# waffcloud/sitewhere

Measured on AMD Instinct MI355X. Metric: device_events_per_sec, higher is better.
Workload: dtype fp64/int64 (event values as in the reference; no reduced precision)

## Files before the change

### csrc/hip/swgpu.hip

```cpp
#include <hip/hip_runtime.h>
#include <hsa/hsa.h>
#include <hsa/hsa_ext_amd.h>
#include <stdint.h>
#include "swtypes.h"
#include "swdecode.h"
#include "swengine.h"
#include "swseg.h"
#include "swblock.h"

#define BLK 256
#define WAVES (BLK / 64)
#define TILE_ITEMS 4
#define TILE (BLK * TILE_ITEMS)
#define MAX_GRID 2048
#define STAGE_BYTES (32 * 1024)
#define MAX_PROBE 4096

#ifndef SW_XCD_REMAP
#define SW_XCD_REMAP 0
#endif
__device__ __forceinline__ uint32_t sw_block_id() {
#if SW_XCD_REMAP
  const uint32_t nwg = gridDim.x, orig = blockIdx.x, x = orig % 8u, q = nwg / 8u, r = nwg % 8u;
  return (x < r ? x * (q + 1u) : r * (q + 1u) + (x - r) * q) + orig / 8u;
// ... 124 lines not shown
}

__device__ __forceinline__ bool stage_window(const uint8_t* __restrict__ raw, const uint32_t* __restrict__ off,
                                             int64_t n_msgs, uint8_t* lds, uint32_t* base_abs) {
  const int64_t m0 = (int64_t)BID * BLK;
  int64_t m1 = m0 + BLK;
  if (m1 > n_msgs) m1 = n_msgs;
  const uint32_t s = off[m0], e = off[m1];
  const uint32_t a0 = s & ~15u;
  const uint32_t span = e - a0;
  if (span > STAGE_BYTES) return false;
  const uint32_t nvec = (span + 15) >> 4;
  const uint4* src = reinterpret_cast<const uint4*>(raw + a0);
  uint4* dst = reinterpret_cast<uint4*>(lds);
  for (uint32_t v = threadIdx.x; v < nvec; v += BLK) dst[v] = src[v];
  __syncthreads();
  *base_abs = a0;
  return true;
}

#define CNT_ERR 0x80000000u
#define CNT_OVR 0x40000000u

__global__ __launch_bounds__(BLK) void k_decode_count(const uint8_t* __restrict__ raw, const uint32_t* __restrict__ off,
                                                      int64_t n_msgs, uint32_t* __restrict__ cnt,
                                                      uint32_t* __restrict__ tsum, SwEngineArgs a) {
  __shared__ __attribute__((aligned(16))) uint8_t lds[STAGE_BYTES];
  if (BID == 0 && threadIdx.x == 0) {
    *a.n_new_names = 0;
    *a.overflow = 0;
    ((ull*)a.stats)[SW_STAT_MSGS] += (ull)a.n_msgs;
  }
  uint32_t base = 0;
  const bool staged = stage_window(raw, off, n_msgs, lds, &base);
  __shared__ uint32_t red[WAVES + 1];
  const int64_t m = (int64_t)BID * BLK + threadIdx.x;
  uint32_t c = 0;
  if (m < n_msgs) {
    uint32_t verdict = SW_DEC_UNKNOWN;
    c = staged ? sw_decode_payload(lds, off[m] - base, off[m + 1] - base, base, 0, 0, nullptr, 0, &verdict)
               : sw_decode_payload(raw, off[m], off[m + 1], 0, 0, 0, nullptr, 0, &verdict);
    cnt[m] = c | (verdict == SW_DEC_ERROR ? CNT_ERR : 0u) | (verdict == SW_DEC_OVERSIZE ? CNT_OVR : 0u);
  }
  uint32_t tot;
  block_excl_scan(c, &tot, red);
  if (threadIdx.x == 0) tsum[BID] = tot;
}

__device__ __forceinline__ void note_name(const SwEventRec& r, ull* __restrict__ key, int64_t mask,
                                          SwNameRef* __restrict__ list, uint32_t* __restrict__ n_list, int64_t cap) {
  if (r.name_hash == 0 || r.etype >= 16) return;
  const ull h = r.name_hash;
  int64_t slot = (int64_t)(h & (ull)mask);
  for (int64_t p = 0; p <= mask && p < MAX_PROBE; ++p) {
    ull old = key[slot];
    if (old == h) return;
    if (old == 0) {
      old = atomicCAS(&key[slot], 0ull, h);
      if (old == 0) {
        const uint32_t k = atomicAdd(n_list, 1u);
        if (k < cap) {
          SwNameRef ref;
          ref.hash = h; ref.off = r.aux_off; ref.len = r.aux_len; ref.src_rank = r.src_rank; ref.pad = r.etype;
          list[k] = ref;
        } else {
          atomicExch(&key[slot], 0ull);
        }
        return;
      }
      if (old == h) return;
    }
    slot = (slot + 1) & mask;
  }
}

__global__ __launch_bounds__(BLK) void k_decode_emit(SwEngineArgs a) {
  __shared__ __attribute__((aligned(16))) uint8_t lds[STAGE_BYTES];
  uint32_t base = 0;
  const bool staged = stage_window(a.raw, a.msg_off, a.n_msgs, lds, &base);
  __shared__ uint32_t red[WAVES + 1];
  const int64_t m = (int64_t)BID * BLK + threadIdx.x;
  uint32_t tot;
  const uint32_t cv = m < a.n_msgs ? a.msg_cnt[m] : 0u;
  const uint32_t pre = block_excl_scan(cv & ~(CNT_ERR | CNT_OVR), &tot, red);
  const uint32_t blk_off = block_sum_prefix(a.msg_evoff, BID, red);
  if (BID == 0) {
    const uint32_t all = block_sum_prefix(a.msg_evoff, gridDim.x, red);
    if (threadIdx.x == 0) *a.n_recs = all;
  }
  if (m >= a.n_msgs) return;
  uint32_t verdict = (cv & CNT_ERR) ? SW_DEC_ERROR : (cv & CNT_OVR) ? SW_DEC_OVERSIZE : SW_DEC_VALID;
  const int64_t o = (int64_t)blk_off + pre;
  if (o >= a.rec_cap) return;
  const uint32_t room = (uint32_t)((a.rec_cap - o) < 0xffffffffll ? (a.rec_cap - o) : 0xffffffffll);
  SwEventRec* out = a.recs + o;
  uint32_t n;
  SwStrRef* sp = a.spans ? a.spans + o : nullptr;
  if (staged)
    n = sw_decode_payload(lds, a.msg_off[m] - base, a.msg_off[m + 1] - base, base, a.now_ms, (uint8_t)a.rank, out, room,
                          &verdict, sp);
// ... 673 lines not shown
      }
    }
    ok += __popcll(__ballot(v && st == SW_ST_OK));
    all += __popcll(__ballot(v));
    if (st != SW_ST_OK) atomicAdd(&rs[st & 7], 1u);
  }
  if (lane_id() == 0) { atomicAdd(&c[0], ok); atomicAdd(&c[1], all - ok); }
  __syncthreads();
  if (threadIdx.x == 0) { tcnt[BID] = c[0]; tcnt[ntiles + BID] = c[1]; }
  if (threadIdx.x < 8 && rs[threadIdx.x]) {
    const int slot = threadIdx.x == SW_ST_UNREGISTERED ? SW_STAT_UNREGISTERED
                   : threadIdx.x == SW_ST_UNASSIGNED ? SW_STAT_UNASSIGNED
                   : threadIdx.x == SW_ST_DUPLICATE ? SW_STAT_DUPLICATE
                   : threadIdx.x == SW_ST_DECODE_ERROR ? SW_STAT_DECODE_ERROR
                   : threadIdx.x == SW_ST_CONTROL ? SW_STAT_CONTROL
                   : threadIdx.x == SW_ST_RECHECK ? SW_STAT_DEDUP_RECHECKS : -1;
    if (slot >= 0) atomicAdd(&stats[slot], (ull)rs[threadIdx.x]);
  }
}

__global__ void k_cmp_write(const uint8_t* __restrict__ status, const uint32_t* __restrict__ n_ptr,
                            const uint32_t* __restrict__ tcnt, int64_t ntiles,
                            uint32_t* __restrict__ ok_idx, uint32_t* __restrict__ rej_idx,
                            uint32_t* __restrict__ n_ok, uint32_t* __restrict__ n_rej) {
  __shared__ uint32_t lds[WAVES + 1];
  const uint32_t n = *n_ptr;
  const int64_t base = (int64_t)BID * TILE;
  uint32_t run_ok = block_sum_prefix(tcnt, BID, lds);
  uint32_t run_rj = block_sum_prefix(tcnt + ntiles, BID, lds);
  if (BID == gridDim.x - 1 && threadIdx.x == 0) {
    *n_ok = run_ok + tcnt[BID];
    *n_rej = run_rj + tcnt[ntiles + BID];
  }
  for (int k = 0; k < TILE_ITEMS; ++k) {
    const int64_t i = base + (int64_t)k * BLK + threadIdx.x;
    const bool valid = i < n;
    const bool ok = valid && status[i] == SW_ST_OK;
    const bool rj = valid && !ok;
    uint32_t tot_ok, tot_rj;
    uint32_t p_ok = block_excl_scan(ok ? 1u : 0u, &tot_ok, lds);
    uint32_t p_rj = block_excl_scan(rj ? 1u : 0u, &tot_rj, lds);
    if (ok) ok_idx[run_ok + p_ok] = (uint32_t)i;
    if (rj) rej_idx[run_rj + p_rj] = (uint32_t)i;
    run_ok += tot_ok;
    run_rj += tot_rj;
  }
}

template <typename K>
__device__ __forceinline__ int64_t nm_probe(const K* __restrict__ key, int64_t mask, ull h) {
  int64_t slot = (int64_t)(h & (ull)mask);
  for (int64_t p = 0; p <= mask && p < MAX_PROBE; ++p) {
    const ull k = key[slot];
    if (k == h) return slot;
    if (k == 0) return -1;
    slot = (slot + 1) & mask;
  }
  return -1;
}

__global__ void k_intern_insert_list(const SwEventRec* __restrict__ recs, const uint32_t* __restrict__ n_ptr,
                                     ull* __restrict__ key, int32_t* __restrict__ ids, int32_t* __restrict__ counter,
                                     int64_t mask, uint32_t cap) {
  const uint32_t n = *n_ptr < cap ? *n_ptr : cap;
  for (int64_t j = (int64_t)BID * BLK + threadIdx.x; j < n; j += (int64_t)gridDim.x * BLK)
    if (recs[j].name_hash) intern_insert(key, ids, counter, mask, recs[j].name_hash);
}

__device__ __forceinline__ int64_t ms_slot(SwMsSlot* __restrict__ ms, int64_t mask, ull k) {
  int64_t slot = (int64_t)(sw_mix64(k) & (ull)mask);
  for (int64_t p = 0; p <= mask && p < MAX_PROBE; ++p) {
    ull* kp = (ull*)&ms[slot].key;
    ull old = *kp;
    if (old == k) return slot;
    if (old == 0) {
      old = atomicCAS(kp, 0ull, k);
      if (old == 0 || old == k) return slot;
    }
    slot = (slot + 1) & mask;
  }
  return -1;
}

__global__ void k_persist(SwEngineArgs a, const SwEventRec* __restrict__ R, const uint32_t* __restrict__ idx,
                          const int32_t* __restrict__ devs, const int32_t* __restrict__ asgs,
                          const uint32_t* __restrict__ n_ptr, uint32_t cap, const SwStrRef* __restrict__ spans,
                          const uint32_t* __restrict__ after) {
  const uint32_t n = *n_ptr < cap ? *n_ptr : cap;
  const int64_t cur = *a.store_cursor + (after ? (int64_t)*after : 0);
  if (idx && BID == 0 && threadIdx.x == 0) {
    if (a.dd_meta[1] + a.rec_cap > (a.dd_mask + 1) / 2) a.dd_meta[2] = 1;
  }
  uint32_t ff_ids = 0;
  const int64_t c0 = *a.step_cursor0;
  const int64_t now = a.sp->now_ms;
  SwSegAux* const aux = reinterpret_cast<SwSegAux*>(a.sp->aux);
  const int64_t raw_bytes = a.sp->raw_bytes;
  for (int64_t j = (int64_t)BID * BLK + threadIdx.x; j < n; j += (int64_t)gridDim.x * BLK) {
    const uint32_t i = idx ? idx[j] : (uint32_t)j;
    const SwEventRec r = R[i];
    const int32_t dev = devs[i], asg = asgs[i];
    const int64_t seq = cur + j;
    const int64_t row = seq % a.store_cap;
    a.s_etype[row] = r.etype;
    a.s_level[row] = r.level;
    a.s_date[row] = r.event_date;
    a.s_recv[row] = now;
    a.s_dev[row] = dev;
    a.s_asg[row] = asg;
    const int4 ctx = *reinterpret_cast<const int4*>(&a.asg_ctx[asg]);
    a.s_cust[row] = ctx.y;
    a.s_area[row] = ctx.z;
    a.s_asset[row] = ctx.w;
    a.s_name[row] = r.name_hash;
    a.s_v0[row] = r.v0;
    a.s_v1[row] = r.v1;
    a.s_v2[row] = r.v2;
    a.s_alt[row] = r.alt_hash;
    a.s_aux[row] = ((ull)r.src_rank << 48) | ((ull)r.aux_len << 32) | (ull)r.aux_off;
    a.s_batch[row] = (int32_t)a.sp->batch_seq;
    SwOutRec o;
    o.event_date = r.event_date;
    o.v0 = r.v0;
    o.v1 = r.v1;
// ... 326 lines not shown
}

__global__ void k_presence(SwEngineArgs a) {
  const SwStepParams P = *a.sp;
  if (P.presence_missing_ms <= 0) return;
  const ull limit = (ull)(P.now_ms - P.presence_missing_ms);
  for (int64_t s = (int64_t)BID * BLK + threadIdx.x; s < a.n_asg; s += (int64_t)gridDim.x * BLK) {
    SwAsgState* st = &a.st[s];
    const ull last = st->last;
    const bool miss = last != 0 && last < limit && st->missing == 0 && a.asg_active[s];
    if (!miss) continue;
    st->missing = (ull)P.now_ms;
    const uint32_t g = atomicAdd(a.n_gen, 1u);
    if (g < a.gen_cap) {
      SwEventRec r;
      r.fp_lo = 0; r.fp_hi = 0; r.event_date = P.now_ms; r.name_hash = a.presence_name_hash;
      r.v0 = 0; r.v1 = 0; r.v2 = 0; r.alt_hash = 0;
      r.aux_off = 0; r.aux2_off = 0; r.aux_len = 0; r.aux2_len = 0;
      r.etype = SW_EV_STATE_CHANGE; r.flags = 0; r.src_rank = (uint8_t)a.rank; r.level = 0;
      a.gen[g] = r;
      a.gen_dev[g] = a.asg_ctx[s].device;
      a.gen_asg[g] = (int32_t)s;
    }
  }
}

__global__ void k_decode_begin(SwEngineArgs a) {
  if (threadIdx.x == 0 && BID == 0) {
    *a.n_new_names = 0;
    *a.overflow = 0;
    ((ull*)a.stats)[SW_STAT_MSGS] += (ull)a.n_msgs;
  }
}

__global__ void k_gen_clamp(SwEngineArgs a, uint32_t* gen_rules) {
  if (threadIdx.x == 0 && BID == 0) {
    if (*a.n_gen > a.gen_cap) *a.n_gen = (uint32_t)a.gen_cap;
    if (gen_rules) *gen_rules = *a.n_gen;
  }
}

__global__ void k_step_end(SwEngineArgs a, const uint32_t* n_rule_alerts) {
  if (threadIdx.x == 0 && BID == 0) {
    if (*a.n_gen > a.gen_cap) *a.n_gen = (uint32_t)a.gen_cap;
    *a.store_cursor += (int64_t)*a.n_ok + *a.n_gen;
    *a.n_out = (uint32_t)(*a.store_cursor - *a.step_cursor0);
    *a.seq_base += *a.n_work;
    ull* st = (ull*)a.stats;
    st[SW_STAT_EVENTS] += *a.n_work;
    st[SW_STAT_PERSISTED] += *a.n_out;
    st[SW_STAT_RULE_ALERTS] += *n_rule_alerts;
    st[SW_STAT_PRESENCE] += *a.n_gen - *n_rule_alerts;
    int64_t* meta = a.dd_meta;
    if (meta[2] == 1) {
// ... 784 lines not shown

int sw_step_snapshot(const uint32_t* scalars, const uint32_t* seg_meta, const uint32_t* rej_cnt,
                     const uint32_t* n_carry, int32_t produced, SwStepSnapshot* host, hipStream_t s) {
  k_step_snapshot<<<1, 64, 0, s>>>(scalars, seg_meta, rej_cnt, n_carry, produced, host);
  return (int)hipGetLastError();
}

int sw_frame_varint(const uint8_t* lens, int64_t nbytes, int64_t n_msgs, uint32_t* msg_off, uint32_t raw_bytes,
                    uint32_t* tmp, int64_t tmp_len, hipStream_t s) {
  int64_t nt = (nbytes + TILE - 1) / TILE;
  if (nt < 1) nt = 1;
  if (2 * nt > tmp_len) return -2;
  if (nbytes <= 0 || n_msgs <= 0) return (int)hipMemsetAsync(msg_off, 0, sizeof(uint32_t) * (n_msgs + 1), s);
  uint32_t* tcnt = tmp;
  uint32_t* tlen = tmp + nt;
  k_vlen_tiles<<<(unsigned)nt, BLK, 0, s>>>(lens, nbytes, tcnt, tlen);
  k_vlen_apply<<<(unsigned)nt, BLK, 0, s>>>(lens, nbytes, tcnt, tlen, msg_off, n_msgs, raw_bytes);
  return (int)hipGetLastError();
}

int sw_phase_decode(const SwEngineArgs* ap, hipStream_t s) {
  const SwEngineArgs a = *ap;
  if (a.n_msgs <= 0) {
    k_decode_begin<<<1, 64, 0, s>>>(a);
    (void)hipMemsetAsync(a.n_recs, 0, sizeof(uint32_t), s);
    return (int)hipGetLastError();
  }
  const unsigned nb = (unsigned)((a.n_msgs + BLK - 1) / BLK);
  k_decode_count<<<nb, BLK, 0, s>>>(a.raw, a.msg_off, a.n_msgs, a.msg_cnt, a.msg_evoff, a);
  k_decode_emit<<<nb, BLK, 0, s>>>(a);
  if (a.world > 1) k_decode_end<<<1, 64, 0, s>>>(a);
  return (int)hipGetLastError();
}

int sw_phase_partition(const SwEngineArgs* ap, hipStream_t s) {
  const SwEngineArgs a = *ap;
  const int64_t ntiles = (a.carry_cap + a.rec_cap + TILE - 1) / TILE;
  if (a.world > 64 || ntiles * a.world > a.part_tmp_len || !a.carry || !a.n_carry || !a.spill || !a.n_spill ||
      a.carry == a.spill || !a.part_owner || !a.part_bytes || !a.part_meta || ntiles >= 0x7fffffff)
    return -3;
  if (a.send_str && (!a.part_len || !a.carry_spans || !a.carry_str || !a.spill_spans || !a.spill_str ||
                     a.carry_str == a.spill_str || a.carry_str_cap <= 0 || a.carry_str_cap > 0xffffffffll ||
                     a.str_cap > 0x7fffffffll))
    return -4;
  k_part_count<<<(unsigned)ntiles, BLK, 0, s>>>(a.carry, a.n_carry, a.recs, a.n_recs, (int)a.world, (int)a.rank,
                                                a.part_tmp, ntiles, a);
  int rc = launch_scan(a.part_tmp, ntiles * a.world, a.part_tmp + ntiles * a.world, nullptr, a.scan_tmp,
                       a.scan_tmp_len, s);
  if (rc) return rc;
  const uint32_t* toff = a.part_tmp + ntiles * a.world;
  k_part_cut<<<(unsigned)a.world, BLK, 0, s>>>(toff, a.part_tmp, ntiles, a.n_carry, a.n_recs, a);
  k_part_write<<<(unsigned)ntiles, BLK, 0, s>>>(a.carry, a.n_carry, a.recs, a.n_recs, (int)a.world, (int)a.rank, toff,
                                                a.part_tmp, ntiles, a.send, a.shuf_cap, a.spill, a.carry_cap, a);
  k_part_counts<<<1, 64, 0, s>>>(toff, a.part_tmp, ntiles, (int)a.world, a);
  return (int)hipGetLastError();
}

int sw_phase_unpack(const SwEngineArgs* ap, hipStream_t s) {
  const SwEngineArgs a = *ap;
  if (a.work_str && (a.str_cap & 15)) return -5;
  k_unpack<<<grid_for(a.rec_cap), BLK, 0, s>>>(a.recv, a.recv_cnt, (int)a.world, a.shuf_cap, a.work, a.n_work,
                                               a.rec_cap, a);
  return (int)hipGetLastError();
}

__global__ void k_cl_prep(const uint32_t* __restrict__ ok_idx, const uint32_t* __restrict__ n_ok,
                          const int32_t* __restrict__ ev_asg, uint32_t* __restrict__ keys, uint32_t* __restrict__ vals) {
  const uint32_t n = *n_ok;
  for (int64_t j = (int64_t)BID * BLK + threadIdx.x; j < n; j += (int64_t)gridDim.x * BLK) {
    const uint32_t i = ok_idx[j];
    keys[j] = (uint32_t)ev_asg[i];
    vals[j] = i;
  }
}

__global__ __launch_bounds__(BLK) void k_ff_add_rows(SwEngineArgs a, const SwEventRec* __restrict__ R,
                                                     const uint32_t* __restrict__ idx,
                                                     const uint32_t* __restrict__ n_ptr, uint32_t cap) {
  if (!a.dd_ff) return;
  const uint32_t n = *n_ptr < cap ? *n_ptr : cap;
  uint32_t* __restrict__ t = a.dd_ff;
  const int gens = (int)a.dd_ff_gens, g = (int)a.dd_ff_meta[0];
  const int64_t bmask = a.dd_ff_bmask;
  const uint32_t lane = threadIdx.x & 63u, sub = lane & 3u, grp = lane >> 2;
  const ull gmask = 0xfull << (4u * grp);
  const int64_t g0 = ((int64_t)BID * BLK + threadIdx.x) >> 2;
  const int64_t gstride = ((int64_t)gridDim.x * BLK) >> 2;
  uint32_t dropped = 0;
  for (int64_t base = g0 - grp; base < (int64_t)n; base += gstride) {
    const int64_t j = base + grp;
    ull h = 0ull;
    if (j < (int64_t)n) h = R[idx ? idx[j] : (uint32_t)j].alt_hash;
    const ull m = sw_ff_mix(h);
    const uint32_t fp = sw_ff_fp(m);
    int64_t b = (int64_t)sw_ff_bucket(m, bmask);
    bool pending = h != 0ull;
    for (int p = 0; p < 2 * SW_FF_MAX_PROBE && __any(pending); ++p) {
      uint32_t* sl = t + (b * gens + g) * SW_FF_SLOTS;
      uint4 v = make_uint4(1u, 1u, 1u, 1u);
      if (pending) v = reinterpret_cast<const uint4*>(sl)[sub];
      const bool hit = pending && (v.x == fp || v.y == fp || v.z == fp || v.w == fp);
      if (__ballot(hit) & gmask) pending = false;
      const bool zero = pending && (!v.x || !v.y || !v.z || !v.w);
      const ull zb = __ballot(zero) & gmask;
      bool ok = false;
      if (pending && zb && lane == (uint32_t)(__ffsll((long long)zb) - 1)) {
        const int k = !v.x ? 0 : !v.y ? 1 : !v.z ? 2 : 3;
        const uint32_t old = atomicCAS(&sl[4u * sub + (uint32_t)k], 0u, fp);
        ok = old == 0u || old == fp;
      }
      if (__ballot(ok) & gmask) pending = false;
      else if (pending && !zb) b = (b + 1) & bmask;
    }
    if (pending && sub == 0u) ++dropped;
  }
  if (dropped) atomicAdd((ull*)&a.dd_ff_meta[5], (ull)dropped);
}

int sw_phase_process(const SwEngineArgs* ap, uint32_t* scratch4, hipStream_t s) {
  const SwEngineArgs a = *ap;
  const int g = grid_for(a.rec_cap);
  const int64_t ntiles = (a.rec_cap + TILE - 1) / TILE;
  if (2 * ntiles > a.scan_tmp_len) return -4;
  if (a.dd_ff && (a.dd_ff_gens < 2 || a.dd_ff_gens > SW_FF_MAX_GENS || !a.dd_ff_meta || a.dd_ff_bmask < 0))
    return -6;
  if (a.n_mtests < 0 || (a.n_mtests > 0 && (!a.mtests || a.n_tests + a.n_mtests > ZONE_LDS_TESTS))) return -7;
  k_lookup<<<g, BLK, 0, s>>>(a);
  if (a.dd_ff) k_ff_probe<<<g, BLK, 0, s>>>(a);
  k_dedup_claim<<<g, BLK, 0, s>>>(a);
  k_cmp_count<<<(unsigned)ntiles, BLK, 0, s>>>(a.status, a.n_work, a.cmp_tmp, ntiles, (ull*)a.stats, a.work,
                                               (const ull*)a.dd_key, a.dd_mask, a.seq_base, a.dd_meta,
                                               a.dd_ff, a.dd_ff_bmask, (int)a.dd_ff_gens, a.work_str ? -1 : (int)a.rank);
  k_cmp_write<<<(unsigned)ntiles, BLK, 0, s>>>(a.status, a.n_work, a.cmp_tmp, ntiles, a.ok_idx, a.rej_idx, a.n_ok,
                                               a.n_rej);
  int rc = 0;
  if (a.cl_bits > 0) {
    k_cl_prep<<<g, BLK, 0, s>>>(a.ok_idx, a.n_ok, a.ev_asg, a.cl_keys, a.cl_vals);
    rc = sw_radix_sort_u32(a.cl_keys, a.cl_vals, a.n_ok, a.rec_cap, (int)a.cl_bits, a.cl_hist, a.ok_idx, s);
    if (rc < 0) return rc;
  }
  const SwStrRef* wsp = a.world > 1 ? a.work_spans : a.spans;
  k_persist<<<g, BLK, 0, s>>>(a, a.work, a.ok_idx, a.ev_dev, a.ev_asg, a.n_ok, (uint32_t)a.rec_cap, wsp, nullptr);
  if (a.dd_ff) k_ff_add_rows<<<g, BLK, 0, s>>>(a, a.work, a.ok_idx, a.n_ok, (uint32_t)a.rec_cap);
  k_state_p2<<<g, BLK, 0, s>>>(a, a.n_ok, (uint32_t)a.rec_cap, nullptr);
  uint32_t* n_rule = scratch4;
  if (a.n_tests + a.n_mtests > 0) {
    const int64_t otiles = (a.rec_cap + TILE - 1) / TILE;
    ull* zmask = (ull*)a.zmask;
    uint32_t* ztile = a.ztile;
    if (a.n_tests > 0) {
      const size_t vtx_bytes = zone_vtx_in_lds(a) ? (size_t)a.n_zone_vtx * 2 * sizeof(double) : 0;
      k_zone_mask<<<(unsigned)otiles, BLK, vtx_bytes, s>>>(a, zmask, ztile);
    }
    if (a.n_mtests > 0) k_mx_mask<<<(unsigned)otiles, BLK, 0, s>>>(a, zmask, ztile, a.n_tests > 0 ? 0 : 1);
    k_zone_emit<<<(unsigned)otiles, BLK, 0, s>>>(a, zmask, ztile, n_rule);
  } else {
    k_gen_clamp<<<1, 64, 0, s>>>(a, n_rule);
  }
  k_presence<<<grid_for(a.n_asg), BLK, 0, s>>>(a);
  const int gg = grid_for(a.gen_cap);
  const uint32_t gcap = (uint32_t)a.gen_cap;
  k_intern_insert_list<<<gg, BLK, 0, s>>>(a.gen, a.n_gen, (ull*)a.nm_key, a.nm_id, a.nm_counter, a.nm_mask, gcap);
  k_persist<<<gg, BLK, 0, s>>>(a, a.gen, nullptr, a.gen_dev, a.gen_asg, a.n_gen, gcap, nullptr, a.n_ok);
  if (a.dd_ff) k_ff_add_rows<<<gg, BLK, 0, s>>>(a, a.gen, nullptr, a.n_gen, gcap);
  k_state_p2<<<gg, BLK, 0, s>>>(a, a.n_gen, gcap, a.n_ok);
  k_step_end<<<1, 64, 0, s>>>(a, n_rule);
  return (int)hipGetLastError();
}

__global__ void k_set_step_params(SwStepParams* sp, int64_t now_ms, int64_t batch_seq, int64_t presence_ms,
                                  SwOutRec* out, void* aux, int64_t raw_bytes) {
  if (threadIdx.x == 0 && BID == 0) {
    sp->now_ms = now_ms; sp->batch_seq = batch_seq; sp->presence_missing_ms = presence_ms; sp->out = out;
    sp->aux = aux; sp->raw_bytes = raw_bytes;
  }
}

__global__ void k_ff_add(uint32_t* t, int64_t bmask, int gens, int g, int64_t* meta, const ull* __restrict__ h,
                         int64_t n) {
  uint32_t dropped = 0;
  for (int64_t i = (int64_t)BID * BLK + threadIdx.x; i < n; i += (int64_t)gridDim.x * BLK)
    if (h[i] && !ff_add(t, bmask, gens, g, h[i])) ++dropped;
  if (dropped) atomicAdd((ull*)&meta[5], (ull)dropped);
}

__global__ void k_ff_clear(uint32_t* t, int64_t bmask, int gens, int g) { ff_clear_gen(t, bmask, gens, g); }

// ... 342 lines not shown
```

### csrc/include/swdecode.h

```cpp
#pragma once
#include "swtypes.h"

SW_HD void sw_fill_control(SwEventRec* r, uint8_t etype, uint32_t abs_start, uint32_t abs_end,
                           uint64_t lo, uint64_t hi, int64_t now_ms, uint8_t src_rank) {
  r->fp_lo = lo; r->fp_hi = hi; r->event_date = now_ms; r->name_hash = 0;
  r->v0 = 0; r->v1 = 0; r->v2 = 0; r->alt_hash = 0;
  r->aux_off = abs_start; r->aux2_off = abs_end; r->aux_len = 0; r->aux2_len = 0;
  r->etype = etype; r->flags = 0; r->src_rank = src_rank; r->level = 0;
}

SW_HD void sw_clear_span(SwStrRef* s) {
  s->alt_off = 0; s->meta_off = 0; s->alt_len = 0; s->meta_len = 0; s->k = 0; s->has = 0; s->pad = 0;
}

SW_HD bool sw_read_tag(const uint8_t* buf, uint32_t* pos, uint32_t end, uint32_t* f, uint32_t* wt) {
  uint64_t key;
  if (!sw_read_varint(buf, pos, end, &key) || key > 0xffffffffull || (key >> 3) == 0) return false;
  *f = (uint32_t)(key >> 3);
  *wt = (uint32_t)(key & 7);
  return true;
}

SW_HD bool sw_check_pair(const uint8_t* buf, uint32_t* pos, uint32_t end, uint32_t wt2, uint32_t* len1 = nullptr) {
  uint64_t len;
// ... 7 lines not shown
    const uint32_t vs = p;
    if (!sw_skip_field(buf, &p, e, wt)) return false;
    if (f == 1 && wt == 2) {
      h1 = true;
      if (len1) {
        uint32_t q = vs;
        uint64_t l;
        sw_read_varint(buf, &q, e, &l);
        if ((uint32_t)l > *len1) *len1 = (uint32_t)l;
      }
    }
    h2 |= f == 2 && wt == wt2;
  }
  *pos = e;
  return h1 && h2;
}

#define SW_DEC_UNKNOWN 0u
#define SW_DEC_VALID 1u
#define SW_DEC_ERROR 2u
#define SW_DEC_OVERSIZE 3u
SW_HD uint32_t sw_decode_payload(const uint8_t* buf, uint32_t start, uint32_t end, uint32_t abs_base,
                                 int64_t now_ms, uint8_t src_rank, SwEventRec* out, uint32_t max_out,
                                 uint32_t* verdict = nullptr, SwStrRef* spans = nullptr) {
  const uint32_t known = verdict ? *verdict : SW_DEC_UNKNOWN;
  if (out && known == SW_DEC_ERROR) {
    if (max_out) {
      sw_fill_control(out, SW_EV_DECODE_ERROR, abs_base + start, abs_base + end, 0, 0, now_ms, src_rank);
      if (spans) sw_clear_span(spans);
    }
    return 1;
  }
  const bool trusted = out && known == SW_DEC_VALID;
  uint32_t pos = start;
  uint64_t hlen = 0, blen = 0, v = 0;
  uint64_t cmd = 0;
  bool ok = sw_read_varint(buf, &pos, end, &hlen) && hlen <= (uint64_t)(end - pos);
  if (ok) {
    uint32_t hend = pos + (uint32_t)hlen;
    while (ok && pos < hend) {
      uint32_t f, wt;
      ok = sw_read_tag(buf, &pos, hend, &f, &wt);
      if (!ok) break;
      if (f == 1 && wt == 0) {
        ok = sw_read_varint(buf, &pos, hend, &v);
        if (v >= 1 && v <= 8) cmd = v;
      } else {
        ok = sw_skip_field(buf, &pos, hend, wt);
      }
    }
    ok = ok && sw_read_varint(buf, &pos, end, &blen) && blen <= (uint64_t)(end - pos);
  }
  if (!ok || cmd < 1 || cmd > 8) {
    if (out && max_out) {
      sw_fill_control(out, SW_EV_DECODE_ERROR, abs_base + start, abs_base + end, 0, 0, now_ms, src_rank);
      if (spans) sw_clear_span(spans);
    }
    if (!out && verdict) *verdict = SW_DEC_ERROR;
    return 1;
  }
  const uint32_t bstart = pos, bend = pos + (uint32_t)blen;
  const bool event = cmd == SW_CMD_SEND_DEVICE_MEASUREMENTS || cmd == SW_CMD_SEND_DEVICE_LOCATION ||
                     cmd == SW_CMD_SEND_DEVICE_ALERT;
  const uint32_t meta_f = cmd == SW_CMD_SEND_DEVICE_MEASUREMENTS ? 4u : cmd == SW_CMD_SEND_DEVICE_LOCATION ? 6u : 5u;

  uint64_t lo = 0, hi = 0, date = 0;
  bool has_dev = false, has_date = false, has_us = false, us = false, has_elev = false, has_alt = false;
  bool req_a = false, req_b = false;
  uint32_t n_mx = 0, name_max = 0;
  double lat = 0, lon = 0, elev = 0;
  uint32_t t_off = start, t_len = 0, m_off = start, m_len = 0;
  uint32_t a_off = start, a_len = 0;
  uint32_t md_lo = 0, md_hi = 0;
  bool has_md = false;
  pos = bstart;
  while (ok && pos < bend) {
    uint32_t f, wt;
    const uint32_t fstart = pos;
    ok = sw_read_tag(buf, &pos, bend, &f, &wt);
    if (!ok) break;
    if (f == 1 && wt == 2) {
// ... 34 lines not shown
          if (f == 2) { lat = d; req_a = true; } else if (f == 3) { lon = d; req_b = true; }
          else if (f == 4) { elev = d; has_elev = true; }
          else { date = bits; has_date = true; }
        } else if (f == 7 && wt == 0) { ok = sw_read_varint(buf, &pos, bend, &v); has_us = true; us = v != 0; }
        else ok = sw_skip_field(buf, &pos, bend, wt);
        break;
      case SW_CMD_SEND_DEVICE_ALERT:
        if ((f == 2 || f == 3) && wt == 2) {
          ok = sw_read_varint(buf, &pos, bend, &v) && v <= (uint64_t)(bend - pos);
          if (!ok) break;
          if (f == 2) { t_off = pos; t_len = (uint32_t)v; req_a = true; } else { m_off = pos; m_len = (uint32_t)v; req_b = true; }
          pos += (uint32_t)v;
        } else if (f == 4 && wt == 1) { if (pos + 8 > bend) { ok = false; break; } date = sw_load_le64(buf + pos); pos += 8; has_date = true; }
        else if (f == 6 && wt == 0) { ok = sw_read_varint(buf, &pos, bend, &v); has_us = true; us = v != 0; }
        else ok = sw_skip_field(buf, &pos, bend, wt);
        break;
      default:
        ok = sw_skip_field(buf, &pos, bend, wt);
        break;
    }
  }
  if ((cmd == SW_CMD_SEND_DEVICE_LOCATION || cmd == SW_CMD_SEND_DEVICE_ALERT) && !(req_a && req_b)) ok = false;
  if (!ok || !has_dev) {
    if (!out && verdict) *verdict = SW_DEC_ERROR;
    if (out && max_out) {
      sw_fill_control(out, SW_EV_DECODE_ERROR, abs_base + start, abs_base + end, 0, 0, now_ms, src_rank);
      if (spans) sw_clear_span(spans);
    }
    return 1;
  }
  const bool oversize = event && (known == SW_DEC_OVERSIZE ||
                                  (!trusted && (a_len > 0xffffu || md_hi - md_lo > 0xffffu || t_len > 0xffffu ||
                                                m_len > 0xffffu || name_max > 0xffffu)));
  if (oversize) {
    if (!out && verdict) *verdict = SW_DEC_OVERSIZE;
    if (!out) return 1;
    if (!max_out) return 0;
    sw_fill_control(out, SW_EV_OVERSIZE, abs_base + start, abs_base + end, lo, hi, now_ms, src_rank);
    if (spans) sw_clear_span(spans);
    return 1;
  }
  uint8_t flags = (has_us ? SW_F_HAS_UPDATE_STATE : 0) | (us ? SW_F_UPDATE_STATE : 0) |
                  (has_date ? SW_F_HAS_DATE : 0) | (has_elev ? SW_F_HAS_ELEVATION : 0);
  int64_t edate = has_date ? (int64_t)date : now_ms;
  SwStrRef sp;
  sp.alt_off = abs_base + a_off; sp.alt_len = (uint16_t)a_len;
  sp.meta_off = has_md ? abs_base + md_lo : abs_base + start; sp.meta_len = has_md ? (uint16_t)(md_hi - md_lo) : 0;
  sp.k = 0; sp.has = (has_alt ? SW_SR_ALT : 0) | (has_md ? SW_SR_META : 0); sp.pad = 0;

  if (!out && verdict) *verdict = SW_DEC_VALID;
  if (!out) return cmd == SW_CMD_SEND_DEVICE_MEASUREMENTS ? n_mx : 1;
  const uint64_t alt = has_alt && (cmd != SW_CMD_SEND_DEVICE_MEASUREMENTS || n_mx == 1) ? sw_hash64(buf + a_off, a_len) : 0;
  if (cmd == SW_CMD_SEND_DEVICE_MEASUREMENTS) {
    if (n_mx > max_out) {
      if (max_out) {
        sw_fill_control(out, SW_EV_DECODE_ERROR, abs_base + start, abs_base + end, lo, hi, now_ms, src_rank);
        if (spans) sw_clear_span(spans);
      }
      return max_out ? 1 : 0;
    }
    const bool multi = n_mx > 1;
    uint32_t k = 0;
    pos = bstart;
    while (pos < bend && k < n_mx) {
      uint64_t key;
      if (!sw_read_varint(buf, &pos, bend, &key)) break;
      uint32_t f = (uint32_t)(key >> 3), wt = (uint32_t)(key & 7);
      if (!(f == 2 && wt == 2)) { if (!sw_skip_field(buf, &pos, bend, wt)) break; continue; }
      sw_read_varint(buf, &pos, bend, &v);
      uint32_t mend = pos + (uint32_t)v;
      uint32_t n_off = start, n_len = 0;
      double val = 0;
      while (pos < mend) {
        uint64_t k2;
// ... 62 lines not shown
```

### csrc/include/swengine.h

```cpp
#pragma once
#include <stddef.h>
#include <stdint.h>
#include "swtypes.h"

typedef struct SwNameRef {
  uint64_t hash;
  uint32_t off;
  uint16_t len;
  uint8_t src_rank;
  uint8_t pad;
} SwNameRef;

typedef struct __attribute__((aligned(16))) SwRegSlot {
  uint64_t lo;
  uint64_t hi;
  int32_t dev;
  int32_t asg;
  uint64_t pad;
} SwRegSlot;

typedef struct __attribute__((aligned(16))) SwAsgCtx {
  int32_t device;
  int32_t customer;
  int32_t area;
// ... 138 lines not shown
  const SwStrRef* recv_spans;
  uint8_t* work_str;
  SwStrRef* work_spans;
  int64_t str_cap;
  uint32_t* str_drops;
  uint8_t* part_owner;
  uint32_t* cl_keys;
  uint32_t* cl_vals;
  uint32_t* cl_hist;
  int64_t cl_bits;
  uint32_t* part_len;
  uint64_t* part_bytes;
  uint64_t* part_meta;
  const SwStrRef* carry_spans;
  const uint8_t* carry_str;
  SwStrRef* spill_spans;
  uint8_t* spill_str;
  uint32_t* n_spill_str;
  int64_t carry_str_cap;
  const SwMxTest* mtests;
  int64_t n_mtests;
} SwEngineArgs;

enum {
  SW_SC_N_RECS = 0,
  SW_SC_N_NEW_NAMES,
  SW_SC_OVERFLOW,
  SW_SC_N_WORK,
  SW_SC_N_OK,
  SW_SC_N_REJ,
  SW_SC_N_GEN,
  SW_SC_N_OUT,
  SW_SC_N_RULE,
  SW_SC_WORDS = 16,
};

typedef struct SwStepSnapshot {
  uint32_t scalars[SW_SC_WORDS];
  uint64_t block_bytes, block_errors, block_first_seq;
  uint32_t n_carry[2];
  uint32_t rej_refs, rej_bytes;
  uint32_t pad[6];
} SwStepSnapshot;
static_assert(sizeof(SwStepSnapshot) == 128, "SwStepSnapshot is 32 u32 words");
static_assert(offsetof(SwStepSnapshot, block_bytes) == 64 && offsetof(SwStepSnapshot, n_carry) == 88 &&
              offsetof(SwStepSnapshot, rej_refs) == 96, "SwStepSnapshot layout");
// ... 139 lines not shown
```

### sitewhere_amd/models/columnar.py

```python
from __future__ import annotations

import numpy as np

EV_MEASUREMENT = 0
EV_LOCATION = 1
EV_ALERT = 2
EV_COMMAND_INVOCATION = 3
EV_COMMAND_RESPONSE = 4
EV_STATE_CHANGE = 5
EV_REGISTRATION = 16
EV_ACK = 17
EV_STREAM_CREATE = 18
EV_STREAM_DATA = 19
EV_STREAM_DATA_REQUEST = 20
EV_DECODE_ERROR = 255

ST_OK = 0
ST_UNREGISTERED = 1
ST_UNASSIGNED = 2
ST_DUPLICATE = 3
ST_DECODE_ERROR = 4
ST_CONTROL = 5
ST_RECHECK = 6

# ... 58 lines not shown

OUT_REC = np.dtype([
    ("event_date", "<i8"), ("v0", "<f8"), ("v1", "<f8"), ("assignment", "<i4"), ("name_id", "<u2"),
    ("etype", "u1"), ("level", "u1"),
])
OUT_REC_SIZE = 32
assert OUT_REC.itemsize == OUT_REC_SIZE
NO_NAME = 0xFFFF

NAME_REF = np.dtype([("hash", "<u8"), ("off", "<u4"), ("len", "<u2"), ("src_rank", "u1"), ("etype", "u1")])
assert NAME_REF.itemsize == 16

REG_SLOT = np.dtype([("lo", "<u8"), ("hi", "<u8"), ("dev", "<i4"), ("asg", "<i4"), ("pad", "<u8")])
assert REG_SLOT.itemsize == 32
ASG_STATE = np.dtype([("last", "<u8"), ("missing", "<u8"), ("loc_date", "<u8"), ("loc_eid1", "<u8")])
MS_SLOT = np.dtype([("key", "<u8"), ("date", "<u8"), ("eid1", "<u8"), ("pad", "<u8")])

ZONE_TEST = np.dtype([("zone", "<i4"), ("condition", "<i4"), ("alert_name_id", "<i4"), ("level", "<i4")])
MX_TEST = np.dtype([("name_hash", "<u8"), ("lo", "<f8"), ("hi", "<f8")])

SC_NAMES = ("n_recs", "n_new_names", "overflow", "n_work", "n_ok", "n_rej", "n_gen", "n_out", "n_rule")
SC_N_RECS, SC_N_NEW_NAMES, SC_OVERFLOW, SC_N_WORK, SC_N_OK, SC_N_REJ, SC_N_GEN, SC_N_OUT, SC_N_RULE = range(9)
SC_WORDS = 16

STEP_SNAPSHOT = np.dtype([
    ("scalars", "<u4", (SC_WORDS,)), ("block_bytes", "<u8"), ("block_errors", "<u8"), ("block_first_seq", "<u8"),
    ("n_carry", "<u4", (2,)), ("rej_refs", "<u4"), ("rej_bytes", "<u4"), ("pad", "<u4", (6,)),
])
assert STEP_SNAPSHOT.itemsize == 128

SERIES_CELL = np.dtype([
    ("count", "<i8"), ("sum", "<f8"), ("min", "<f8"), ("max", "<f8"), ("first", "<f8"), ("last", "<f8"),
    ("first_date", "<i8"), ("last_date", "<i8"), ("first_id", "<i8"), ("last_id", "<i8"),
])
assert SERIES_CELL.itemsize == 80
SERIES_MAX_NAMES = 64
SERIES_MAX_CELLS = 65536
RING_QUERY = ("etype", "asg", "date", "n_rows", "seq0", "head", "bits", "n_asg", "start", "end")
SERIES_QUERY = RING_QUERY + ("name", "v0", "names", "n_names", "bucket_ms", "n_buckets", "rounds", "grid")
NEAR_QUERY = RING_QUERY + ("v0", "v1", "lat", "lon", "radius_m", "lat_lo", "lat_hi", "lon_lo", "lon_hi", "latest",
                           "best_date", "best_seq")
NEAR_QUERY_F64 = ("lat", "lon", "radius_m", "lat_lo", "lat_hi", "lon_lo", "lon_hi")
ZONE_QUERY = RING_QUERY + ("v0", "v1", "vtx", "n_vtx", "lat_lo", "lat_hi", "lon_lo", "lon_hi", "outside", "latest",
                           "best_date", "best_seq")
ZONE_QUERY_F64 = ("lat_lo", "lat_hi", "lon_lo", "lon_hi")
GRID_CELL = np.dtype([("count", "<i8"), ("last_date", "<i8")])
# ... 30 lines not shown
```

### sitewhere_amd/pipeline/gpu_engine.py

```python
from __future__ import annotations

import ctypes
import functools
import os
import time

import numpy as np
import torch

from .._native import gpu_gil as gpu_lib
from ..models.columnar import (EVENT_REC, RANK_CELL, RANK_QUERY, GRID_CELL, GRID_QUERY_F64, GRID_WORDS, N_STATS, NEAR_QUERY, NEAR_QUERY_F64,
                               OUT_REC, NAME_REF, OUT_REC_SIZE, RING_QUERY, SC_N_GEN, SC_N_NEW_NAMES, SC_N_OK, SC_N_OUT,
                               SC_N_RECS, SC_N_REJ, SC_N_RULE, SC_N_WORK, SC_NAMES, SC_OVERFLOW, SEG_ST_BYTES, SEG_ST_FIRST, SEG_ST_WORDS, SERIES_CELL, SERIES_QUERY,
                               ST_RECHECK, STEP_SNAPSHOT, STR_REF, WIRE_REC, ZONE_QUERY, ZONE_QUERY_F64)
from ..ops.engine_abi import SwEngineArgs
from .config import EngineConfig
from .bus_io import host_view
from .engine_base import EngineBase, StepResult
from .pinned_pool import PinnedPool

_ALIGN = 64
_I64 = np.iinfo(np.int64)


def _ptr(t: torch.Tensor) -> int:
    return t.data_ptr()


def _chk(rc: int, name: str):
    if rc:
        raise RuntimeError(f"{name} failed ({rc})")


class HostBuffer:
# ... 541 lines not shown
        return self.t["recv"][q * n:(q + 1) * n]

    def loopback_strings(self, peers: list):
        c = self.cfg
        if not c.str_cap:
            return
        sr = c.shuf_cap * STR_REF.itemsize
        q = self.rank
        for r, e in enumerate(peers):
            p = e._last_send_par
            self.t["recv_str_cnt"][r] = e.send_str_cnts[p][q]
            self.t["recv_spans"][r * sr:(r + 1) * sr].copy_(e.send_spans[p][q * sr:(q + 1) * sr])
            self.t["recv_str"][r * c.str_cap:(r + 1) * c.str_cap].copy_(
                e.send_strs[p][q * c.str_cap:(q + 1) * c.str_cap])

    def string_drops(self) -> dict:
        v = self.t["str_drops"].cpu().numpy()
        return {"oversize": int(v[0])}

    def scalars(self) -> dict:
        v = self.t["scalars"][:len(SC_NAMES)].cpu().numpy()
        return {name: int(x) for name, x in zip(SC_NAMES, v)}

    def step(self, raw: np.ndarray, offs: np.ndarray, now_ms: int, presence: bool | None = None) -> StepResult:
        n_msgs = len(offs) - 1
        with self._lock:
            self._no_framed_pending()
            raw_dev, off_dev = self._stage(raw, offs)
            do_presence = self.presence_due(now_ms) if presence is None else presence
            sel = self.step_async(raw_dev, off_dev, n_msgs, now_ms, presence=do_presence, out_to_device=True)
            self._sync_streams()
            return self._with_block(self.collect(sel, raw, from_device=True), sel, now_ms)

    def decode_only(self, raw: np.ndarray, offs: np.ndarray, now_ms: int, spans: bool = False):
        n_msgs = len(offs) - 1
        with self._lock:
            self._no_framed_pending()
            raw_dev, off_dev = self._stage(raw, offs)
            self._set_batch(raw_dev, off_dev, n_msgs, now_ms)
            _chk(self.lib.sw_phase_decode(ctypes.byref(self.args), self._stream()), "sw_phase_decode")
            self._sync_streams()
            n = min(int(self.t["scalars"][SC_N_RECS].item()), self.cfg.rec_cap)
            recs = self.t["recs"][:n * EVENT_REC.itemsize].cpu().numpy().view(EVENT_REC).copy()
            if not spans:
                return recs
            return recs, self.t["spans"][:n * STR_REF.itemsize].cpu().numpy().view(STR_REF).copy()
# ... 1159 lines not shown
```

Before: 523.4 million.

## Speculate single-event decode in one pass and fold cluster prep into compaction

Decoding now speculates that every message yields exactly one event. The first kernel decodes straight into the output records and only runs the two-pass emit kernel when some block saw a message with a different count. A small mode state machine on the device tracks recent fallbacks across batches so later batches use the classic path after one misses. Separately, the cluster key/value preparation kernel is merged into the compaction write, persist reads the sorted assignment keys directly, and the generated-event bloom-add launch is dropped in favour of reading alt hashes back from the store ring. These changes cut a full decode pass and several launches per step, at the cost of extra state and wasted speculative work when a batch contains multi-event messages.

```diff
diff --git a/csrc/hip/swgpu.hip b/csrc/hip/swgpu.hip
--- a/csrc/hip/swgpu.hip
+++ b/csrc/hip/swgpu.hip
@@ -170,30 +170,7 @@
 #define CNT_ERR 0x80000000u
 #define CNT_OVR 0x40000000u
 
-__global__ __launch_bounds__(BLK) void k_decode_count(const uint8_t* __restrict__ raw, const uint32_t* __restrict__ off,
-                                                      int64_t n_msgs, uint32_t* __restrict__ cnt,
-                                                      uint32_t* __restrict__ tsum, SwEngineArgs a) {
-  __shared__ __attribute__((aligned(16))) uint8_t lds[STAGE_BYTES];
-  if (BID == 0 && threadIdx.x == 0) {
-    *a.n_new_names = 0;
-    *a.overflow = 0;
-    ((ull*)a.stats)[SW_STAT_MSGS] += (ull)a.n_msgs;
-  }
-  uint32_t base = 0;
-  const bool staged = stage_window(raw, off, n_msgs, lds, &base);
-  __shared__ uint32_t red[WAVES + 1];
-  const int64_t m = (int64_t)BID * BLK + threadIdx.x;
-  uint32_t c = 0;
-  if (m < n_msgs) {
-    uint32_t verdict = SW_DEC_UNKNOWN;
-    c = staged ? sw_decode_payload(lds, off[m] - base, off[m + 1] - base, base, 0, 0, nullptr, 0, &verdict)
-               : sw_decode_payload(raw, off[m], off[m + 1], 0, 0, 0, nullptr, 0, &verdict);
-    cnt[m] = c | (verdict == SW_DEC_ERROR ? CNT_ERR : 0u) | (verdict == SW_DEC_OVERSIZE ? CNT_OVR : 0u);
-  }
-  uint32_t tot;
-  block_excl_scan(c, &tot, red);
-  if (threadIdx.x == 0) tsum[BID] = tot;
-}
+__device__ __forceinline__ uint32_t* dec_mode(const SwEngineArgs& a) { return a.n_recs + SW_SC_DECODE_MODE; }
 
 __device__ __forceinline__ void note_name(const SwEventRec& r, ull* __restrict__ key, int64_t mask,
                                           SwNameRef* __restrict__ list, uint32_t* __restrict__ n_list, int64_t cap) {
@@ -222,8 +199,62 @@
   }
 }
 
+__global__ void k_decode_begin(SwEngineArgs a, int classic) {
+  if (threadIdx.x == 0 && BID == 0) {
+    *a.n_new_names = 0;
+    *a.overflow = 0;
+    ((ull*)a.stats)[SW_STAT_MSGS] += (ull)a.n_msgs;
+    uint32_t* dm = dec_mode(a);
+    const uint32_t k = dm[SW_DM_BATCH] + 1u;
+    dm[SW_DM_BATCH] = k;
+    const bool cl = classic || dm[SW_DM_FORCE] || dm[SW_DM_W0 + (k + 2u) % 3u];
+    dm[SW_DM_W0 + (k + 1u) % 3u] = 0;
+    dm[SW_DM_MODE] = cl ? 1u : 0u;
+    if (!cl) ++dm[SW_DM_SPECULATED];
+  }
+}
+
+__global__ __launch_bounds__(BLK) void k_decode_first(SwEngineArgs a) {
+  __shared__ __attribute__((aligned(16))) uint8_t lds[STAGE_BYTES];
+  uint32_t base = 0;
+  const bool staged = stage_window(a.raw, a.msg_off, a.n_msgs, lds, &base);
+  __shared__ uint32_t red[WAVES + 1];
+  const uint32_t* dm = dec_mode(a);
+  const bool classic = dm[SW_DM_MODE] != 0u;
+  const int64_t m = (int64_t)BID * BLK + threadIdx.x;
+  uint32_t c = 0;
+  bool other = false;
+  if (m < a.n_msgs) {
+    uint32_t verdict = SW_DEC_UNKNOWN;
+    const uint32_t s = a.msg_off[m], e = a.msg_off[m + 1];
+    if (classic) {
+      c = staged ? sw_decode_payload(lds, s - base, e - base, base, 0, 0, nullptr, 0, &verdict)
+                 : sw_decode_payload(a.raw, s, e, 0, 0, 0, nullptr, 0, &verdict);
+    } else {
+      SwEventRec* out = a.recs + m;
+      SwStrRef* sp = a.spans ? a.spans + m : nullptr;
+      if (staged) sw_decode_payload(lds, s - base, e - base, base, a.now_ms, (uint8_t)a.rank, out, 1, &verdict, sp, &c);
+      else sw_decode_payload(a.raw, s, e, 0, a.now_ms, (uint8_t)a.rank, out, 1, &verdict, sp, &c);
+      if (c == 1u) note_name(*out, (ull*)a.seen_key, a.seen_mask, a.new_names, a.n_new_names, a.names_cap);
+    }
+    other = c != 1u;
+    a.msg_cnt[m] = c | (verdict == SW_DEC_ERROR ? CNT_ERR : 0u) | (verdict == SW_DEC_OVERSIZE ? CNT_OVR : 0u);
+  }
+  uint32_t tot;
+  block_excl_scan(c, &tot, red);
+  if (threadIdx.x == 0) a.msg_evoff[BID] = tot;
+  if (!classic && BID == 0 && threadIdx.x == 0) *a.n_recs = (uint32_t)a.n_msgs;
+  if (__syncthreads_or(other) && threadIdx.x == 0) dec_mode(a)[SW_DM_W0 + dm[SW_DM_BATCH] % 3u] = 1u;
+}
+
 __global__ __launch_bounds__(BLK) void k_decode_emit(SwEngineArgs a) {
   __shared__ __attribute__((aligned(16))) uint8_t lds[STAGE_BYTES];
+  {
+    uint32_t* dm = dec_mode(a);
+    const bool classic = dm[SW_DM_MODE] != 0u;
+    if (!classic && !dm[SW_DM_W0 + dm[SW_DM_BATCH] % 3u]) return;
+    if (!classic && BID == 0 && threadIdx.x == 0) ++dm[SW_DM_FALLBACKS];
+  }
   uint32_t base = 0;
   const bool staged = stage_window(a.raw, a.msg_off, a.n_msgs, lds, &base);
   __shared__ uint32_t red[WAVES + 1];
@@ -943,7 +974,9 @@
 __global__ void k_cmp_write(const uint8_t* __restrict__ status, const uint32_t* __restrict__ n_ptr,
                             const uint32_t* __restrict__ tcnt, int64_t ntiles,
                             uint32_t* __restrict__ ok_idx, uint32_t* __restrict__ rej_idx,
-                            uint32_t* __restrict__ n_ok, uint32_t* __restrict__ n_rej) {
+                            uint32_t* __restrict__ n_ok, uint32_t* __restrict__ n_rej,
+                            const int32_t* __restrict__ ev_asg, uint32_t* __restrict__ cl_keys,
+                            uint32_t* __restrict__ cl_vals) {
   __shared__ uint32_t lds[WAVES + 1];
   const uint32_t n = *n_ptr;
   const int64_t base = (int64_t)BID * TILE;
@@ -961,7 +994,14 @@
     uint32_t tot_ok, tot_rj;
     uint32_t p_ok = block_excl_scan(ok ? 1u : 0u, &tot_ok, lds);
     uint32_t p_rj = block_excl_scan(rj ? 1u : 0u, &tot_rj, lds);
-    if (ok) ok_idx[run_ok + p_ok] = (uint32_t)i;
+    if (ok) {
+      if (cl_keys) {
+        cl_keys[run_ok + p_ok] = (uint32_t)ev_asg[i];
+        cl_vals[run_ok + p_ok] = (uint32_t)i;
+      } else {
+        ok_idx[run_ok + p_ok] = (uint32_t)i;
+      }
+    }
     if (rj) rej_idx[run_rj + p_rj] = (uint32_t)i;
     run_ok += tot_ok;
     run_rj += tot_rj;
@@ -1006,7 +1046,7 @@
 __global__ void k_persist(SwEngineArgs a, const SwEventRec* __restrict__ R, const uint32_t* __restrict__ idx,
                           const int32_t* __restrict__ devs, const int32_t* __restrict__ asgs,
                           const uint32_t* __restrict__ n_ptr, uint32_t cap, const SwStrRef* __restrict__ spans,
-                          const uint32_t* __restrict__ after) {
+                          const uint32_t* __restrict__ after, const uint32_t* __restrict__ sorted_asg) {
   const uint32_t n = *n_ptr < cap ? *n_ptr : cap;
   const int64_t cur = *a.store_cursor + (after ? (int64_t)*after : 0);
   if (idx && BID == 0 && threadIdx.x == 0) {
@@ -1020,7 +1060,7 @@
   for (int64_t j = (int64_t)BID * BLK + threadIdx.x; j < n; j += (int64_t)gridDim.x * BLK) {
     const uint32_t i = idx ? idx[j] : (uint32_t)j;
     const SwEventRec r = R[i];
-    const int32_t dev = devs[i], asg = asgs[i];
+    const int32_t dev = devs[i], asg = sorted_asg ? (int32_t)sorted_asg[j] : asgs[i];
     const int64_t seq = cur + j;
     const int64_t row = seq % a.store_cap;
     a.s_etype[row] = r.etype;
@@ -1393,14 +1433,6 @@
       a.gen_dev[g] = a.asg_ctx[s].device;
       a.gen_asg[g] = (int32_t)s;
     }
-  }
-}
-
-__global__ void k_decode_begin(SwEngineArgs a) {
-  if (threadIdx.x == 0 && BID == 0) {
-    *a.n_new_names = 0;
-    *a.overflow = 0;
-    ((ull*)a.stats)[SW_STAT_MSGS] += (ull)a.n_msgs;
   }
 }
 
@@ -2231,12 +2263,13 @@
 int sw_phase_decode(const SwEngineArgs* ap, hipStream_t s) {
   const SwEngineArgs a = *ap;
   if (a.n_msgs <= 0) {
-    k_decode_begin<<<1, 64, 0, s>>>(a);
+    k_decode_begin<<<1, 64, 0, s>>>(a, 1);
     (void)hipMemsetAsync(a.n_recs, 0, sizeof(uint32_t), s);
     return (int)hipGetLastError();
   }
   const unsigned nb = (unsigned)((a.n_msgs + BLK - 1) / BLK);
-  k_decode_count<<<nb, BLK, 0, s>>>(a.raw, a.msg_off, a.n_msgs, a.msg_cnt, a.msg_evoff, a);
+  k_decode_begin<<<1, 64, 0, s>>>(a, a.rec_cap < a.n_msgs ? 1 : 0);
+  k_decode_first<<<nb, BLK, 0, s>>>(a);
   k_decode_emit<<<nb, BLK, 0, s>>>(a);
   if (a.world > 1) k_decode_end<<<1, 64, 0, s>>>(a);
   return (int)hipGetLastError();
@@ -2273,21 +2306,12 @@
   return (int)hipGetLastError();
 }
 
-__global__ void k_cl_prep(const uint32_t* __restrict__ ok_idx, const uint32_t* __restrict__ n_ok,
-                          const int32_t* __restrict__ ev_asg, uint32_t* __restrict__ keys, uint32_t* __restrict__ vals) {
-  const uint32_t n = *n_ok;
-  for (int64_t j = (int64_t)BID * BLK + threadIdx.x; j < n; j += (int64_t)gridDim.x * BLK) {
-    const uint32_t i = ok_idx[j];
-    keys[j] = (uint32_t)ev_asg[i];
-    vals[j] = i;
-  }
-}
-
 __global__ __launch_bounds__(BLK) void k_ff_add_rows(SwEngineArgs a, const SwEventRec* __restrict__ R,
                                                      const uint32_t* __restrict__ idx,
                                                      const uint32_t* __restrict__ n_ptr, uint32_t cap) {
   if (!a.dd_ff) return;
   const uint32_t n = *n_ptr < cap ? *n_ptr : cap;
+  const int64_t cur = *a.store_cursor;
   uint32_t* __restrict__ t = a.dd_ff;
   const int gens = (int)a.dd_ff_gens, g = (int)a.dd_ff_meta[0];
   const int64_t bmask = a.dd_ff_bmask;
@@ -2299,7 +2323,7 @@
   for (int64_t base = g0 - grp; base < (int64_t)n; base += gstride) {
     const int64_t j = base + grp;
     ull h = 0ull;
-    if (j < (int64_t)n) h = R[idx ? idx[j] : (uint32_t)j].alt_hash;
+    if (j < (int64_t)n) h = R ? R[idx[j]].alt_hash : a.s_alt[(cur + j) % a.store_cap];
     const ull m = sw_ff_mix(h);
     const uint32_t fp = sw_ff_fp(m);
     int64_t b = (int64_t)sw_ff_bucket(m, bmask);
@@ -2340,17 +2364,22 @@
   k_cmp_count<<<(unsigned)ntiles, BLK, 0, s>>>(a.status, a.n_work, a.cmp_tmp, ntiles, (ull*)a.stats, a.work,
                                                (const ull*)a.dd_key, a.dd_mask, a.seq_base, a.dd_meta,
                                                a.dd_ff, a.dd_ff_bmask, (int)a.dd_ff_gens, a.work_str ? -1 : (int)a.rank);
+  const bool cluster = a.cl_bits > 0;
   k_cmp_write<<<(unsigned)ntiles, BLK, 0, s>>>(a.status, a.n_work, a.cmp_tmp, ntiles, a.ok_idx, a.rej_idx, a.n_ok,
-                                               a.n_rej);
-  int rc = 0;
-  if (a.cl_bits > 0) {
-    k_cl_prep<<<g, BLK, 0, s>>>(a.ok_idx, a.n_ok, a.ev_asg, a.cl_keys, a.cl_vals);
-    rc = sw_radix_sort_u32(a.cl_keys, a.cl_vals, a.n_ok, a.rec_cap, (int)a.cl_bits, a.cl_hist, a.ok_idx, s);
+                                               a.n_rej, a.ev_asg, cluster ? a.cl_keys : nullptr, a.cl_vals);
+  const uint32_t* sorted_asg = nullptr;
+  if (cluster) {
+    const int rc = sw_radix_sort_u32(a.cl_keys, a.cl_vals, a.n_ok, a.rec_cap, (int)a.cl_bits, a.cl_hist, a.ok_idx, s);
     if (rc < 0) return rc;
+    sorted_asg = a.cl_keys + (int64_t)rc * a.rec_cap;
   }
   const SwStrRef* wsp = a.world > 1 ? a.work_spans : a.spans;
-  k_persist<<<g, BLK, 0, s>>>(a, a.work, a.ok_idx, a.ev_dev, a.ev_asg, a.n_ok, (uint32_t)a.rec_cap, wsp, nullptr);
-  if (a.dd_ff) k_ff_add_rows<<<g, BLK, 0, s>>>(a, a.work, a.ok_idx, a.n_ok, (uint32_t)a.rec_cap);
+  k_persist<<<g, BLK, 0, s>>>(a, a.work, a.ok_idx, a.ev_dev, a.ev_asg, a.n_ok, (uint32_t)a.rec_cap, wsp, nullptr,
+                              sorted_asg);
+  if (a.dd_ff) {
+    const bool ring = a.store_cap >= a.rec_cap;
+    k_ff_add_rows<<<g, BLK, 0, s>>>(a, ring ? nullptr : a.work, a.ok_idx, a.n_ok, (uint32_t)a.rec_cap);
+  }
   k_state_p2<<<g, BLK, 0, s>>>(a, a.n_ok, (uint32_t)a.rec_cap, nullptr);
   uint32_t* n_rule = scratch4;
   if (a.n_tests + a.n_mtests > 0) {
@@ -2370,8 +2399,7 @@
   const int gg = grid_for(a.gen_cap);
   const uint32_t gcap = (uint32_t)a.gen_cap;
   k_intern_insert_list<<<gg, BLK, 0, s>>>(a.gen, a.n_gen, (ull*)a.nm_key, a.nm_id, a.nm_counter, a.nm_mask, gcap);
-  k_persist<<<gg, BLK, 0, s>>>(a, a.gen, nullptr, a.gen_dev, a.gen_asg, a.n_gen, gcap, nullptr, a.n_ok);
-  if (a.dd_ff) k_ff_add_rows<<<gg, BLK, 0, s>>>(a, a.gen, nullptr, a.n_gen, gcap);
+  k_persist<<<gg, BLK, 0, s>>>(a, a.gen, nullptr, a.gen_dev, a.gen_asg, a.n_gen, gcap, nullptr, a.n_ok, nullptr);
   k_state_p2<<<gg, BLK, 0, s>>>(a, a.n_gen, gcap, a.n_ok);
   k_step_end<<<1, 64, 0, s>>>(a, n_rule);
   return (int)hipGetLastError();
diff --git a/csrc/include/swdecode.h b/csrc/include/swdecode.h
--- a/csrc/include/swdecode.h
+++ b/csrc/include/swdecode.h
@@ -53,8 +53,11 @@
 #define SW_DEC_OVERSIZE 3u
 SW_HD uint32_t sw_decode_payload(const uint8_t* buf, uint32_t start, uint32_t end, uint32_t abs_base,
                                  int64_t now_ms, uint8_t src_rank, SwEventRec* out, uint32_t max_out,
-                                 uint32_t* verdict = nullptr, SwStrRef* spans = nullptr) {
+                                 uint32_t* verdict = nullptr, SwStrRef* spans = nullptr,
+                                 uint32_t* full_cnt = nullptr) {
   const uint32_t known = verdict ? *verdict : SW_DEC_UNKNOWN;
+  const bool report = verdict && (!out || (full_cnt && known == SW_DEC_UNKNOWN));
+  if (full_cnt) *full_cnt = 1;
   if (out && known == SW_DEC_ERROR) {
     if (max_out) {
       sw_fill_control(out, SW_EV_DECODE_ERROR, abs_base + start, abs_base + end, 0, 0, now_ms, src_rank);
@@ -87,7 +90,7 @@
       sw_fill_control(out, SW_EV_DECODE_ERROR, abs_base + start, abs_base + end, 0, 0, now_ms, src_rank);
       if (spans) sw_clear_span(spans);
     }
-    if (!out && verdict) *verdict = SW_DEC_ERROR;
+    if (report) *verdict = SW_DEC_ERROR;
     return 1;
   }
   const uint32_t bstart = pos, bend = pos + (uint32_t)blen;
@@ -168,7 +171,7 @@
   }
   if ((cmd == SW_CMD_SEND_DEVICE_LOCATION || cmd == SW_CMD_SEND_DEVICE_ALERT) && !(req_a && req_b)) ok = false;
   if (!ok || !has_dev) {
-    if (!out && verdict) *verdict = SW_DEC_ERROR;
+    if (report) *verdict = SW_DEC_ERROR;
     if (out && max_out) {
       sw_fill_control(out, SW_EV_DECODE_ERROR, abs_base + start, abs_base + end, 0, 0, now_ms, src_rank);
       if (spans) sw_clear_span(spans);
@@ -179,7 +182,7 @@
                                   (!trusted && (a_len > 0xffffu || md_hi - md_lo > 0xffffu || t_len > 0xffffu ||
                                                 m_len > 0xffffu || name_max > 0xffffu)));
   if (oversize) {
-    if (!out && verdict) *verdict = SW_DEC_OVERSIZE;
+    if (report) *verdict = SW_DEC_OVERSIZE;
     if (!out) return 1;
     if (!max_out) return 0;
     sw_fill_control(out, SW_EV_OVERSIZE, abs_base + start, abs_base + end, lo, hi, now_ms, src_rank);
@@ -194,8 +197,9 @@
   sp.meta_off = has_md ? abs_base + md_lo : abs_base + start; sp.meta_len = has_md ? (uint16_t)(md_hi - md_lo) : 0;
   sp.k = 0; sp.has = (has_alt ? SW_SR_ALT : 0) | (has_md ? SW_SR_META : 0); sp.pad = 0;
 
-  if (!out && verdict) *verdict = SW_DEC_VALID;
+  if (report) *verdict = SW_DEC_VALID;
   if (!out) return cmd == SW_CMD_SEND_DEVICE_MEASUREMENTS ? n_mx : 1;
+  if (full_cnt && cmd == SW_CMD_SEND_DEVICE_MEASUREMENTS) *full_cnt = n_mx;
   const uint64_t alt = has_alt && (cmd != SW_CMD_SEND_DEVICE_MEASUREMENTS || n_mx == 1) ? sw_hash64(buf + a_off, a_len) : 0;
   if (cmd == SW_CMD_SEND_DEVICE_MEASUREMENTS) {
     if (n_mx > max_out) {
diff --git a/csrc/include/swengine.h b/csrc/include/swengine.h
--- a/csrc/include/swengine.h
+++ b/csrc/include/swengine.h
@@ -184,6 +184,17 @@
   int64_t n_mtests;
 } SwEngineArgs;
 
+#define SW_SC_DECODE_MODE 32
+enum {
+  SW_DM_BATCH = 0,
+  SW_DM_W0 = 1,
+  SW_DM_MODE = 4,
+  SW_DM_FORCE = 5,
+  SW_DM_SPECULATED = 6,
+  SW_DM_FALLBACKS = 7,
+  SW_DM_WORDS = 8,
+};
+
 enum {
   SW_SC_N_RECS = 0,
   SW_SC_N_NEW_NAMES,
diff --git a/sitewhere_amd/models/columnar.py b/sitewhere_amd/models/columnar.py
--- a/sitewhere_amd/models/columnar.py
+++ b/sitewhere_amd/models/columnar.py
@@ -104,6 +104,8 @@
 SC_NAMES = ("n_recs", "n_new_names", "overflow", "n_work", "n_ok", "n_rej", "n_gen", "n_out", "n_rule")
 SC_N_RECS, SC_N_NEW_NAMES, SC_OVERFLOW, SC_N_WORK, SC_N_OK, SC_N_REJ, SC_N_GEN, SC_N_OUT, SC_N_RULE = range(9)
 SC_WORDS = 16
+DECODE_MODE = 32
+DM_FORCE, DM_SPECULATED, DM_FALLBACKS, DM_WORDS = 5, 6, 7, 8
 
 STEP_SNAPSHOT = np.dtype([
     ("scalars", "<u4", (SC_WORDS,)), ("block_bytes", "<u8"), ("block_errors", "<u8"), ("block_first_seq", "<u8"),
diff --git a/sitewhere_amd/pipeline/gpu_engine.py b/sitewhere_amd/pipeline/gpu_engine.py
--- a/sitewhere_amd/pipeline/gpu_engine.py
+++ b/sitewhere_amd/pipeline/gpu_engine.py
@@ -9,7 +9,7 @@
 import torch
 
 from .._native import gpu_gil as gpu_lib
-from ..models.columnar import (EVENT_REC, RANK_CELL, RANK_QUERY, GRID_CELL, GRID_QUERY_F64, GRID_WORDS, N_STATS, NEAR_QUERY, NEAR_QUERY_F64,
+from ..models.columnar import (DECODE_MODE, DM_FALLBACKS, DM_FORCE, DM_SPECULATED, DM_WORDS, EVENT_REC, RANK_CELL, RANK_QUERY, GRID_CELL, GRID_QUERY_F64, GRID_WORDS, N_STATS, NEAR_QUERY, NEAR_QUERY_F64,
                                OUT_REC, NAME_REF, OUT_REC_SIZE, RING_QUERY, SC_N_GEN, SC_N_NEW_NAMES, SC_N_OK, SC_N_OUT,
                                SC_N_RECS, SC_N_REJ, SC_N_RULE, SC_N_WORK, SC_NAMES, SC_OVERFLOW, SEG_ST_BYTES, SEG_ST_FIRST, SEG_ST_WORDS, SERIES_CELL, SERIES_QUERY,
                                ST_RECHECK, STEP_SNAPSHOT, STR_REF, WIRE_REC, ZONE_QUERY, ZONE_QUERY_F64)
@@ -597,6 +597,15 @@
         v = self.t["scalars"][:len(SC_NAMES)].cpu().numpy()
         return {name: int(x) for name, x in zip(SC_NAMES, v)}
 
+    def decode_mode(self) -> tuple:
+        self._sync_streams()
+        v = self.t["scalars"][DECODE_MODE:DECODE_MODE + DM_WORDS].cpu().numpy()
+        return int(v[DM_SPECULATED]), int(v[DM_FALLBACKS])
+
+    def force_classic_decode(self, on: bool = True):
+        self._sync_streams()
+        self.t["scalars"][DECODE_MODE + DM_FORCE] = int(bool(on))
+
     def step(self, raw: np.ndarray, offs: np.ndarray, now_ms: int, presence: bool | None = None) -> StepResult:
         n_msgs = len(offs) - 1
         with self._lock:
```

Measured after the change: 479.5 million. 0.916x the previous value.
